# 0xmenna/spmv-scpa

Hardware: AMD Instinct MI355X
Metric: fp64 SpMV GFLOP/s + achieved HBM GB/s (% of roofline), 1/2/4/8 MI355X (higher is better)
Workload: dtype f64

## Files before the change

### include/spmv_engine.h

```cpp
#ifndef SPMV_ENGINE_H
#define SPMV_ENGINE_H

#include <stddef.h>
#include <stdint.h>

#include "csr.h"
#include "hll.h"

#ifdef __cplusplus
extern "C" {
#endif

typedef struct spmv_launch_opts {
    int waves_per_block;
    int group;
    int variant;
    int reserved[5];
} spmv_launch_opts;

int spmv_device_count(void);
int spmv_set_device(int device);
int spmv_get_device(void);
int spmv_device_info(int device, char *name, size_t len, int *compute_units,
                     size_t *hbm_bytes);
// ... 229 lines not shown
                      const spmv_trsv_plan *second, const double *d_scale,
                      double tol, int maxit, int check_every, void *d_work,
                      size_t work_bytes, spmv_cg_info *info, void *stream);

int64_t spmv_bicgstab_work_bytes(int M, int k);
int spmv_csr_bicgstab(const spmv_csr_dev *A, const spmv_launch_opts *opts,
                      int k, const double *d_B, int64_t ldb, double *d_X,
                      int64_t ldx, const double *d_minv,
                      double tol, int maxit, int check_every,
                      void *d_work, size_t work_bytes,
                      spmv_cg_info *info, void *stream);
int spmv_hll_bicgstab(const spmv_hll_dev *H, const spmv_launch_opts *opts,
                      int k, const double *d_B, int64_t ldb, double *d_X,
                      int64_t ldx, const double *d_minv,
                      double tol, int maxit, int check_every,
                      void *d_work, size_t work_bytes,
                      spmv_cg_info *info, void *stream);

typedef struct spmv_cgls_info {
    int status;
    int iterations;
    double ss;
    double atb;
    double rr;
} spmv_cgls_info;

int64_t spmv_cgls_work_bytes(int M, int N, int k);
int spmv_csr_cgls(const spmv_csr_dev *A, const spmv_csr_dev *AT,
                  const spmv_launch_opts *opts, int k,
                  const double *d_B, int64_t ldb, double *d_X, int64_t ldx,
                  double damp, double tol, int maxit, int check_every,
                  void *d_work, size_t work_bytes,
                  spmv_cgls_info *info, void *stream);
int spmv_hll_cgls(const spmv_hll_dev *H, const spmv_hll_dev *HT,
                  const spmv_launch_opts *opts, int k,
                  const double *d_B, int64_t ldb, double *d_X, int64_t ldx,
                  double damp, double tol, int maxit, int check_every,
                  void *d_work, size_t work_bytes,
                  spmv_cgls_info *info, void *stream);

typedef struct spmv_minres_info {
    int status;
    int iterations;
    double pp;
    double bn2;
    double rr;
    double bb;
} spmv_minres_info;

int64_t spmv_minres_work_bytes(int M, int k);
int spmv_csr_minres(const spmv_csr_dev *A, const spmv_launch_opts *opts, int k,
                    const double *d_B, int64_t ldb, double *d_X, int64_t ldx,
                    const double *d_minv, double tol, int maxit,
                    int check_every, void *d_work, size_t work_bytes,
                    spmv_minres_info *info, void *stream);
int spmv_hll_minres(const spmv_hll_dev *H, const spmv_launch_opts *opts, int k,
                    const double *d_B, int64_t ldb, double *d_X, int64_t ldx,
                    const double *d_minv, double tol, int maxit,
                    int check_every, void *d_work, size_t work_bytes,
                    spmv_minres_info *info, void *stream);
int spmv_debug_sqrt(const double *d_in, double *d_out, int64_t n, void *stream);

int spmv_csr_autotune(spmv_csr_dev *A, const double *d_x, double *d_y,
                      int allow_panels, int *best_kernel, double *best_ms);
int spmv_hll_autotune(spmv_hll_dev *H, const double *d_x, double *d_y,
                      int allow_panels, int *best_kernel, double *best_ms);

int spmv_csr_tune_times(const spmv_csr_dev *A, double *ms, int n);
int spmv_hll_tune_times(const spmv_hll_dev *H, double *ms, int n);
int spmv_csr_tune_log(const spmv_csr_dev *A, char *buf, size_t len);
int spmv_hll_tune_log(const spmv_hll_dev *H, char *buf, size_t len);

int spmv_live_handles(void);
long spmv_ignored_releases(void);
void spmv_set_debug(int on);
uint64_t spmv_handle_generation(const void *handle);
void spmv_csr_release_checked(spmv_csr_dev *A, uint64_t generation);
void spmv_hll_release_checked(spmv_hll_dev *H, uint64_t generation);

const char *spmv_version(void);
int spmv_csr_debug_stale_arrivals(spmv_csr_dev *A);
int spmv_hll_debug_stale_arrivals(spmv_hll_dev *H);

int spmv_hip_build_version(void);
int spmv_hip_runtime_version(void);
const char *spmv_build_flavour(void);

#ifdef __cplusplus
}
#endif
#endif
```

### spmv_scpa_amd/csrc/engine.hip

```cpp
#include <algorithm>
#include <cmath>
#include <functional>
#include <mutex>
#include <stdio.h>
#include <stdlib.h>
#include <string.h>
#include <string>
#include <thread>
#include <time.h>
#include <unordered_map>
#include <vector>

#include "err.h"
#include "hip_common.h"
#include "hip_csr.h"
#include "hip_hll.h"
#include "mat_ref.h"
#include "spmv_synth.h"
#include "stream_table.h"
#include "transpose_plan.h"
#include "trsv_plan.h"
#include "tune_blocked.h"
#include "utils.h"

// ... 51 lines not shown
    } while (0)

struct panels_ops {
    static void free(spmv_panels *p) { panels_free(p); }
    static void set_chain(spmv_panels *p, int v) { panels_set_chain(p, v); }
    static void set_waves(spmv_panels *p, int v) { panels_set_waves(p, v); }
    static void set_order(spmv_panels *p, int v) { panels_set_order(p, v); }
    static int balanced_tile_rows(int M, int max_rows) {
        return panels_balanced_tile_rows(M, max_rows);
    }
    static const char *build_phases(void) { return panels_last_build_phases(); }
    static double now_s(void) {
        struct timespec t;
        clock_gettime(CLOCK_MONOTONIC, &t);
        return (double)t.tv_sec + 1e-9 * (double)t.tv_nsec;
    }
};

struct tune_log {
    std::string text;
    void operator()(const char *line) {
        text += line;
        text += '\n';
    }
    char *release(void) const { return strdup(text.c_str()); }
};

extern "C" {

const char *spmv_version(void) { return "spmv_scpa_amd 0.7 gfx950"; }

int spmv_hip_build_version(void) { return HIP_VERSION; }
int spmv_hip_runtime_version(void) {
    int v = 0;
    return hipRuntimeGetVersion(&v) == hipSuccess ? v : -EIO;
}

const char *spmv_build_flavour(void) {
#ifdef SPMV_ABLATIONS
    return "ablations";
#else
    return "product";
#endif
}

int spmv_live_handles(void) {
    std::lock_guard<std::mutex> g(live().mu);
    return (int)live().handles.size();
}

long spmv_ignored_releases(void) {
    std::lock_guard<std::mutex> g(live().mu);
    return live().ignored;
}

void spmv_set_debug(int on) {
    std::lock_guard<std::mutex> g(live().mu);
    live().debug = on ? 1 : 0;
}

uint64_t spmv_handle_generation(const void *handle) {
    std::lock_guard<std::mutex> g(live().mu);
    auto it = live().handles.find(handle);
    return it == live().handles.end() ? 0 : it->second;
}

static int stale_arrivals(unsigned long long *cnt, int n, spmv_panels *P) {
    if (cnt && n > 0)
        HIP_RET(hipMemset(cnt, 0x01, (size_t)n * sizeof(unsigned long long)));
    else
        n = 0;
    const int p = panels_debug_stale_arrivals(P);
    return p < 0 ? p : n + p;
}

int spmv_csr_debug_stale_arrivals(spmv_csr_dev *A) {
    HANDLE_OK(A);
    return stale_arrivals(A->seg_count, A->n_rowblk, A->panels);
}

int spmv_hll_debug_stale_arrivals(spmv_hll_dev *H) {
    HANDLE_OK(H);
    return stale_arrivals(H->wide_cnt, H->n_wide_seg, H->panels);
}

void set_csr_waves_per_block(int waves) {
    g_csr_waves = waves < 1 ? 0 : (waves > 16 ? 16 : waves);
}

void set_hll_waves_per_block(int waves) {
    g_hll_waves = waves < 1 ? 0 : (waves > 16 ? 16 : waves);
}


int spmv_device_count(void) {
    int n = 0;
    if (hipGetDeviceCount(&n) != hipSuccess)
        return 0;
    return n;
}

int spmv_set_device(int device) {
    if (spmv_device_count() == 0)
        return -ENODEV;
    HIP_RET(hipSetDevice(device));
    return 0;
}

int spmv_get_device(void) {
    int d = 0;
    if (spmv_device_count() == 0)
        return -ENODEV;
    HIP_RET(hipGetDevice(&d));
    return d;
}

int spmv_device_info(int device, char *name, size_t len, int *compute_units,
                     size_t *hbm_bytes) {
    if (spmv_device_count() == 0)
        return -ENODEV;
    hipDeviceProp_t p;
    HIP_RET(hipGetDeviceProperties(&p, device));
    if (name && len)
        snprintf(name, len, "%s (%s)", p.name, p.gcnArchName);
    if (compute_units)
        *compute_units = p.multiProcessorCount;
    if (hbm_bytes)
        *hbm_bytes = p.totalGlobalMem;
    return 0;
}

int spmv_device_pci_bus_id(int device, char *buf, size_t len) {
    if (!buf || len < 16)
        return -EINVAL;
    if (spmv_device_count() == 0)
        return -ENODEV;
    HIP_RET(hipDeviceGetPCIBusId(buf, (int)len, device));
    return 0;
}

int spmv_dev_mem_info(size_t *free_bytes, size_t *total_bytes) {
    if (spmv_device_count() == 0)
        return -ENODEV;
    size_t f = 0, t = 0;
    HIP_RET(hipMemGetInfo(&f, &t));
    if (free_bytes)
        *free_bytes = f;
    if (total_bytes)
        *total_bytes = t;
    return 0;
}

int spmv_dev_malloc(void **dptr, size_t bytes) {
    if (!dptr)
        return -EINVAL;
    *dptr = NULL;
    if (spmv_device_count() == 0)
        return -ENODEV;
    HIP_RET(hipMalloc(dptr, bytes ? bytes : 16));
    return 0;
}

int spmv_dev_free(void *dptr) {
    if (!dptr)
        return 0;
    HIP_RET(hipFree(dptr));
// ... 2920 lines not shown
```

### spmv_scpa_amd/csrc/hip_common.h

```cpp
#ifndef SPMV_HIP_COMMON_H
#define SPMV_HIP_COMMON_H

#include <errno.h>
#include <hip/hip_runtime.h>
#include <stdint.h>
#include <type_traits>

#include "spmv_engine.h"

#define WAVE 64
#define NUM_XCD 8
#define XCD_GROUP 32
#define HACK HACK_SIZE

static inline unsigned grouped_grid(unsigned n) {
    return (n + NUM_XCD * XCD_GROUP - 1) / (NUM_XCD * XCD_GROUP) * NUM_XCD *
           XCD_GROUP;
}

static inline int hip_errno(hipError_t e) {
    switch (e) {
    case hipSuccess:
        return 0;
    case hipErrorNoDevice:
// ... 353 lines not shown
int bicgstab_solve(const cg_matrix *A, int k, const double *B, int64_t ldb,
                   double *X, int64_t ldx, const double *minv, double tol,
                   int maxit, int check_every, void *d_work, size_t work_bytes,
                   spmv_cg_info *info, hipStream_t s);

int64_t cgls_work_bytes(int M, int N, int k);
int cgls_solve(const cg_matrix *A, const cg_matrix *AT, int k, const double *B,
               int64_t ldb, double *X, int64_t ldx, double damp, double tol,
               int maxit, int check_every, void *d_work, size_t work_bytes,
               spmv_cgls_info *info, hipStream_t s);

int64_t minres_work_bytes(int M, int k);
int minres_solve(const cg_matrix *A, int k, const double *B, int64_t ldb,
                 double *X, int64_t ldx, const double *minv, double tol,
                 int maxit, int check_every, void *d_work, size_t work_bytes,
                 spmv_minres_info *info, hipStream_t s);
int minres_debug_sqrt(const double *d_in, double *d_out, int64_t n,
                      hipStream_t s);

int csr_diag(const spmv_csr_dev *A, double *out, int invert, hipStream_t s);
int hll_diag(const spmv_hll_dev *H, double *out, int invert, hipStream_t s);

int csr_transpose_dev(const spmv_csr_dev *A, spmv_csr_dev *T, hipStream_t s);
int csr_equal_dev(const spmv_csr_dev *X, const spmv_csr_dev *Y, int *pattern,
                  int *values, hipStream_t s);
void tr_scan(int *data, int64_t n, int *sums, hipStream_t s);

struct trsv_segment;
struct spmv_trsv_plan {
    int M, uplo, unit, levels, value_bytes, device;
    int widest_level;
    int64_t entries;
    int64_t zero_diag;
    int64_t bytes;
    int *level;
    int *order;
    int *level_ptr;
    int *rowptr;
    int *ja;
    void *as;
    double *diag;
    int *h_level_ptr;
    trsv_segment *segs;
    int n_segs;
};
int trsv_analyse_dev(const spmv_csr_dev *A, int uplo, int unit, int max_levels,
                     spmv_trsv_plan *P, hipStream_t s);
void trsv_free_dev(spmv_trsv_plan *P);
int trsv_solve_dev(const spmv_trsv_plan *P, int waves, int k, const double *B,
                   int64_t ldb, double *X, int64_t ldx, const double *scale,
                   hipStream_t s);

typedef int (*ic0_alloc_fn)(int M, int N, int64_t NZ, int value_bytes,
                            spmv_csr_dev **out);
int ic0_factor_dev(const spmv_csr_dev *A, double shift, int max_levels,
                   int waves, ic0_alloc_fn alloc, spmv_csr_dev **out,
                   spmv_ic0_info *info, hipStream_t s);

int csr_launch_kernel(const spmv_csr_dev *A, int kernel, int waves, int group,
                      int variant, const double *x, double *y, int r0, int r1,
                      hipStream_t s);
int hll_launch_kernel(const spmv_hll_dev *H, int kernel, int waves,
                      int variant, const double *x, double *y, int b0, int b1,
                      hipStream_t s);
int hll_fix_pads_dev(spmv_hll_dev *H, hipStream_t s);
int hll16_convert_dev(const spmv_hll_dev *src, spmv_hll_dev *dst,
                      unsigned *d_overflow, hipStream_t s);

int panels_from_csr(const spmv_csr_dev *A, int panel_cols, int sched,
                    int tile_rows, spmv_panels **out);
int panels_from_hll(const spmv_hll_dev *H, int panel_cols, int sched,
                    int tile_rows, spmv_panels **out);
int panels_from_csr_opts(const spmv_csr_dev *A, const spmv_panel_opts *o,
                         spmv_panels **out);
int panels_from_hll_opts(const spmv_hll_dev *H, const spmv_panel_opts *o,
                         spmv_panels **out);
void panels_get_opts(const spmv_panels *P, spmv_panel_opts *o);
int panels_is_sweep(const spmv_panels *P);
int panels_tile_rows(const spmv_panels *P);
int panels_is_chain(const spmv_panels *P);
void panels_set_chain(spmv_panels *P, int chain);
void panels_set_waves(spmv_panels *P, int waves);
int panels_debug_stale_arrivals(spmv_panels *P);
void panels_set_order(spmv_panels *P, int order);
int panels_waves(const spmv_panels *P);
void panels_fit_steps(const spmv_panels *P, int64_t *builtin, int64_t *fit);
void panels_set_fit_steps(spmv_panels *P, int64_t builtin, int64_t fit);
int panels_plan_kernel(const spmv_panels *P, int waves, int variant,
                       int *threads, int *groups, int *ordered);
int panels_launch(const spmv_panels *P, int M, int waves, int variant,
                  const double *x, double *y, hipStream_t s);
void panels_free(spmv_panels *p);
int64_t panels_nnz(const spmv_panels *P);
int panels_count(const spmv_panels *P);
int panels_steps(const spmv_panels *P);
int panels_tiles(const spmv_panels *P);
int panels_balanced_tile_rows(int M, int max_rows);
int panels_describe(const spmv_panels *P, char *buf, size_t len);
const char *panels_last_build_phases(void);
void panels_pool_begin(void);
void panels_pool_end(void);

extern int g_csr_waves;
extern int g_hll_waves;

#endif
```

### spmv_scpa_amd/csrc/panels.hip

```cpp
#include <algorithm>
#include <atomic>
#include <utility>
#include <hipcub/hipcub.hpp>
#include <stdio.h>
#include <string.h>
#include <vector>

#include <time.h>

#include "hip_common.h"
#include "panel_launch.h"
#include "panel_build.h"

#define SWEEP_SPIN_MAX 512
#define CNT_STRIDE 32
#define SWEEP_TAIL 16384

struct spmv_panels : panel_shape {
    int N;
    int shift;
    int reserve_cus;
    int pmajor;
    int64_t total;
    unsigned *ent;
    double *val;
    int64_t *bptr;
    int *blen;
    int64_t *cb;
    int *cpanel;
    int *nbk;
    int span;
    int residue;
    int bucket_order;
    int xcd_first[NUM_XCD + 1];
    int *phase_cnt;
    size_t phase_cnt_bytes;
    int nlong;
    int nlong_seg;
    int64_t long_nnz;
    int *long_row;
    int *long_ptr;
    int *long_ja;
    double *long_as;
    int2 *long_seg;
    int *long_seg0;
    double *long_part;
    unsigned long long *long_cnt;
    unsigned launch_epoch;
};

static hipError_t big_malloc(void **p, size_t bytes);
static void big_free(void *p);

template <bool POOLED> struct dev_block {
    void *p = NULL;
    dev_block() = default;
    dev_block(dev_block &&o) : p(o.p) { o.p = NULL; }
    dev_block &operator=(dev_block &&o) {
        std::swap(p, o.p);
        return *this;
    }
    ~dev_block() { reset(); }
    hipError_t alloc(size_t bytes) {
        return POOLED ? big_malloc(&p, bytes) : hipMalloc(&p, bytes);
    }
    void reset() {
        if (POOLED)
            big_free(p);
        else
            (void)hipFree(p);
        p = NULL;
    }
    template <typename T> T *as() const { return (T *)p; }
};
typedef dev_block<true> pooled_block;
typedef dev_block<false> plain_block;

void panels_free(spmv_panels *p) {
    if (!p)
        return;
    big_free(p->ent);
    big_free(p->val);
    (void)hipFree(p->cpanel);
    (void)hipFree(p->phase_cnt);
    (void)hipFree(p->bptr);
    (void)hipFree(p->blen);
    (void)hipFree(p->cb);
    (void)hipFree(p->nbk);
    (void)hipFree(p->long_row);
    (void)hipFree(p->long_ptr);
    (void)hipFree(p->long_ja);
    (void)hipFree(p->long_as);
    (void)hipFree(p->long_seg);
    (void)hipFree(p->long_seg0);
    (void)hipFree(p->long_part);
    (void)hipFree(p->long_cnt);
    free(p);
}

__host__ __device__ __forceinline__ uint64_t bucket_id(uint64_t tile,
                                                       uint64_t panel,
                                                       uint64_t panels,
                                                       uint64_t pm_grid) {
    return pm_grid ? ((tile / pm_grid) * panels + panel) * pm_grid + tile % pm_grid
                   : tile * panels + panel;
}

__device__ __forceinline__ bool in_sorted(const int *__restrict__ rows, int n,
                                          int row) {
    int lo = 0, hi = n;
    while (lo < hi) {
        const int mid = (lo + hi) >> 1;
        if (rows[mid] < row)
            lo = mid + 1;
        else
            hi = mid;
    }
    return lo < n && rows[lo] == row;
}
// ... 675 lines not shown

static int compact_lists(const panel_geometry &g, spmv_panels *P,
                         plain_block &span_block) {
    const int tiles = g.tiles, panels = g.panels;
    HIP_RET(hipMalloc((void **)&P->cb,
                      ((size_t)g.nbuckets + 1) * 2 * sizeof(int64_t)));
    HIP_RET(hipMalloc((void **)&P->cpanel,
                      ((size_t)g.nbuckets + 1) * sizeof(int)));
    HIP_RET(hipMalloc((void **)&P->nbk, ((size_t)tiles + 1) * sizeof(int)));
    HIP_RET(hipMemset(P->nbk, 0, ((size_t)tiles + 1) * sizeof(int)));
    if (tiles > 0) {
        HIP_RET(span_block.alloc((2 * (size_t)tiles + 1) * sizeof(int)));
        int *span = span_block.as<int>();
        HIP_RET(hipMemset(span + 2 * (size_t)tiles, 0, sizeof(int)));
        hipLaunchKernelGGL(k_tile_span, dim3((tiles + 255) / 256), dim3(256), 0,
                           0, tiles, panels, P->blen, span, span + tiles,
                           span + 2 * (size_t)tiles);
        HIP_RET(hipGetLastError());
        HIP_RET(hipMemcpy(&P->span, span + 2 * (size_t)tiles, sizeof(int),
                          hipMemcpyDeviceToHost));
        P->residue = P->bucket_order != 1 && P->span > 1 && P->span < panels;
        hipLaunchKernelGGL(k_compact_buckets, dim3((tiles + 255) / 256),
                           dim3(256), 0, 0, tiles, panels,
                           P->residue ? P->span : panels, P->bptr, P->blen, span,
                           span + tiles, P->cb, P->cpanel, P->nbk);
        hipLaunchKernelGGL(k_max_int, dim3(64), dim3(256), 0, 0, tiles, P->nbk,
                           P->nbk + tiles);
        HIP_RET(hipGetLastError());
    }
    HIP_RET(hipMemcpy(&P->max_nbk, P->nbk + tiles, sizeof(int),
                      hipMemcpyDeviceToHost));
    return 0;
}

static int bucket_totals(const panel_geometry &g, const int64_t *raw,
                         spmv_panels *P) {
    HIP_RET(hipMemcpy(&P->nnz, raw + g.nbuckets, sizeof(int64_t),
                      hipMemcpyDeviceToHost));
    HIP_RET(hipMemcpy(&P->total, P->bptr + g.nbuckets, sizeof(int64_t),
                      hipMemcpyDeviceToHost));
    return P->total + SWEEP_TAIL > (int64_t)3000000000LL ? -EOVERFLOW : 0;
}

static int place_entries(const panel_geometry &g, const uint64_t *skey,
                         const double *sval, const int64_t *raw,
                         spmv_panels *P) {
    const size_t m = (size_t)P->total + SWEEP_TAIL;
    HIP_RET(big_malloc((void **)&P->ent, m * sizeof(unsigned)));
    HIP_RET(big_malloc((void **)&P->val, m * sizeof(double)));
    HIP_RET(hipMemset(P->ent, 0, m * sizeof(unsigned)));
    HIP_RET(hipMemset(P->val, 0, m * sizeof(double)));
    if (P->nnz > 0) {
        const unsigned grid = (unsigned)((P->nnz + 255) / 256);
        hipLaunchKernelGGL(k_place, dim3(grid), dim3(256), 0, 0, P->nnz, g.shift,
                           g.rbits, skey, sval, raw, P->bptr, P->ent, P->val);
        HIP_RET(hipGetLastError());
        HIP_RET(hipDeviceSynchronize());
    }
    return 0;
}

static int count_chunk_steps(const panel_geometry &g, spmv_panels *P) {
    P->fit_steps[0] = P->fit_steps[1] = 0;
    panel_plan pl;
    if (g.nbuckets <= 0 || P->nnz <= 0 ||
        panel_launch_plan(*P, 0, 0, false, &pl) || pl.family != PANEL_SWEEP)
        return 0;
    plain_block sums;
    HIP_RET(sums.alloc(2 * sizeof(unsigned long long)));
    HIP_RET(hipMemset(sums.p, 0, 2 * sizeof(unsigned long long)));
    hipLaunchKernelGGL(k_chunk_steps, dim3(64), dim3(256), 0, 0,
                       (int64_t)g.nbuckets, P->blen, pl.k.threads * pl.k.q * 4,
                       PANEL_FIT_CHUNK, sums.as<unsigned long long>());
    HIP_RET(hipGetLastError());
    unsigned long long h[2] = {0, 0};
    HIP_RET(hipMemcpy(h, sums.p, sizeof h, hipMemcpyDeviceToHost));
    P->fit_steps[0] = (int64_t)h[0];
    P->fit_steps[1] = (int64_t)h[1];
    return 0;
}

static int alloc_phase_counters(const panel_geometry &g, spmv_panels *P) {
    const size_t rounds = ((size_t)g.tiles + g.grid - 1) / g.grid;
    P->phase_cnt_bytes = NUM_XCD * (rounds ? rounds : 1) * (size_t)g.panels *
                         CNT_STRIDE * sizeof(int);
    HIP_RET(hipMalloc((void **)&P->phase_cnt, P->phase_cnt_bytes));
    return 0;
}

struct build_scratch {
    pooled_block key[2], sv[2];
    pooled_block idx;
    pooled_block tmp;
    pooled_block flag;
    plain_block count;
    plain_block raw, padded;
    plain_block span;
    ~build_scratch() {
        for (int k = 0; k < 2; ++k) {
            key[k].reset();
            sv[k].reset();
        }
        idx.reset();
        tmp.reset();
        flag.reset();
        count.reset();
        raw.reset();
        padded.reset();
        span.reset();
    }
};

static int build_stages(const panel_geometry &g, const build_src &s,
                        spmv_panels *P) {
    int rc;
    build_scratch b;
    const bool hll = !s.irp;
    int64_t n_sort = s.slots;
    uint64_t *skey;
    double *sval;
    double tp[5] = {build_now_s(), 0, 0, 0, 0};

    if ((rc = long_rows_extract(P, s)))
        return rc;
    if (hll && s.slots > 0 &&
        (rc = hll_flag_kept(s, P, b.flag, b.count, &n_sort)))
        return rc;
    if ((rc = alloc_sort_buffers(n_sort, hll && n_sort != s.slots, b.key, b.sv,
                                 b.idx)))
        return rc;
    skey = b.key[0].as<uint64_t>();
    sval = b.sv[0].as<double>();
    if (s.slots > 0) {
        rc = hll ? keys_from_hll(g, s, n_sort, b.flag, b.count, b.idx, skey, sval)
                 : keys_from_csr(g, s, P, skey, sval);
        if (rc)
            return rc;
        tp[1] = build_now_s();
        b.idx.reset();
        if ((rc = sort_keys(g, n_sort, b.key, b.sv, b.tmp, &skey, &sval)))
            return rc;
    }
    tp[2] = build_now_s();
    if ((rc = bucket_tables(g, n_sort, skey, P, b.raw, b.padded)))
        return rc;
    if (!g.sweep && (rc = compact_lists(g, P, b.span)))
        return rc;
    if ((rc = bucket_totals(g, b.raw.as<int64_t>(), P)))
        return rc;
    tp[3] = build_now_s();
    if ((rc = place_entries(g, skey, sval, b.raw.as<int64_t>(), P)))
        return rc;
    if ((rc = g.sweep ? alloc_phase_counters(g, P) : balance_xcd_ranges(P)))
        return rc;
    if (g.sweep && (rc = count_chunk_steps(g, P)))
        return rc;
    tp[4] = build_now_s();
    snprintf(g_build_phases, sizeof g_build_phases,
             "%lld of %lld slots sorted: alloc+keys %.3f s, sort %.3f, bucket "
             "tables %.3f, place %.3f",
             (long long)n_sort, (long long)s.slots,
             tp[1] > 0 ? tp[1] - tp[0] : 0.0, tp[1] > 0 ? tp[2] - tp[1] : 0.0,
             tp[3] - tp[2], tp[4] - tp[3]);
    return 0;
}

static int panels_build(int N, const build_src &s, const spmv_panel_opts *o,
                        spmv_panels **out) {
    *out = NULL;
    spmv_panel_opts dflt;
    spmv_panel_opts_default(&dflt);
    if (!o)
        o = &dflt;
    long long tall_rows = 0;
#ifdef SPMV_ABLATIONS
    if (const char *e = getenv("SPMV_ABL_SWEEP_TILE_ROWS")) {
        const long long v = atoll(e) / 32 * 32;
        if (v >= 32 && v < (1 << 20))
            tall_rows = v;
    }
#endif
    panel_geometry g;
    int rc = panel_build_plan(s.M, N, s.slots, *o,
                              g_panel_sched.load(std::memory_order_relaxed),
                              device_cus, tall_rows, &g);
    if (rc)
        return rc;
    spmv_panels *P = (spmv_panels *)calloc(1, sizeof *P);
    if (!P)
        return -ENOMEM;
    P->N = N;
    P->shift = g.shift;
    P->panels = g.panels;
    P->tile_rows = g.tile_rows;
    P->tiles = g.tiles;
    P->sweep = g.sweep;
    P->chain = g.chain;
    P->grid = g.grid;
    P->wgs_per_cu = g.wgs_per_cu;
    P->reserve_cus = g.reserve_cus;
    P->pmajor = g.pmajor;
    P->lds_min = o->lds_min;
    P->bucket_order = o->bucket_order;
    P->det = g.det;
    P->order = g.order;
    g_build_phases[0] = 0;
    rc = build_stages(g, s, P);
    if (rc) {
        panels_free(P);
        return rc;
    }
    *out = P;
    return 0;
}

__device__ __forceinline__ void phase_arrive(int *cnt, int n = 1) {
    __hip_atomic_fetch_add(cnt, n, __ATOMIC_RELAXED, __HIP_MEMORY_SCOPE_AGENT);
}

__device__ __forceinline__ bool phase_wait(const int *cnt, int want, int spin) {
    for (int i = 0; i < spin; ++i) {
        if (__hip_atomic_load(cnt, __ATOMIC_RELAXED, __HIP_MEMORY_SCOPE_AGENT) >=
            want)
            return true;
        __builtin_amdgcn_s_sleep(8);
    }
    return false;
}

#define WAVE_RING 32
__device__ __forceinline__ void wg_arrive(int *ring, int q, int waves,
                                          int *cnt_q) {
    const int old = atomicAdd(&ring[q & (WAVE_RING - 1)], 1);
    if (old == waves - 1) {
        atomicExch(&ring[q & (WAVE_RING - 1)], 0);
        phase_arrive(cnt_q);
    }
}

typedef unsigned u32x4 __attribute__((ext_vector_type(4)));
typedef double f64x2 __attribute__((ext_vector_type(2)));


#ifndef SPMV_DET_SLEEP
#define SPMV_DET_SLEEP 1
#endif
__device__ __forceinline__ void det_wait(int *turn, int want) {
    while (__hip_atomic_load(turn, __ATOMIC_ACQUIRE,
                             __HIP_MEMORY_SCOPE_WORKGROUP) != want) {
#if SPMV_DET_SLEEP > 0
        __builtin_amdgcn_s_sleep(SPMV_DET_SLEEP);
#endif
    }
}

__device__ __forceinline__ void det_have(double v) {
    asm volatile("" ::"v"(v));
}

__device__ __forceinline__ void det_pass(int *turn, int next) {
    __hip_atomic_store(turn, next, __ATOMIC_RELEASE,
                       __HIP_MEMORY_SCOPE_WORKGROUP);
}

template <int Q> struct sweep_chunk {
    u32x4 en[Q];
    f64x2 va[Q], vb[Q];
    int live[Q];
    int p;
    int pa;
    bool first, last;
};

template <int NT, int Q, int ABL = 0, bool DET = false>
__global__ void __launch_bounds__(NT)
    k_tiles_sweep(int M, int tile_rows, int tiles, int panels, int shift,
                  int lag, int spin, int stagger, int pmajor, unsigned total,
                  const int64_t *__restrict__ bptr,
                  const int *__restrict__ blen,
                  const unsigned *__restrict__ tent,
                  const double *__restrict__ tval,
                  const double *__restrict__ x, double *__restrict__ y,
                  int *phase_cnt) {
    extern __shared__ double ytile[];
    __shared__ int wave_done[WAVE_RING];
    constexpr int WAVES = NT / WAVE;
    constexpr unsigned CH = NT * Q * 4;
    const int tid = threadIdx.x;
    const int grid = gridDim.x;
    const int xcd = blockIdx.x % NUM_XCD;
    const int n_x = grid / NUM_XCD + (xcd < (grid % NUM_XCD) ? 1 : 0);
    const int rounds = (tiles + grid - 1) / grid;
    int *cnt = phase_cnt + (size_t)xcd * rounds * panels * CNT_STRIDE;
    const unsigned lowmask = (ABL & 2) ? 1023u : (1u << shift) - 1u;
    __shared__ int det_turn;
    int det_seq = tid / WAVE;
    if (tid < WAVE_RING)
        wave_done[tid] = 0;
    if (tid == 0)
        det_turn = 0;
    bool synced = true;

    for (int r = 0; r < rounds; ++r) {
        const int t = r * grid + blockIdx.x;
        const int q0 = r * panels;
        if (t >= tiles) {
            if (tid == 0)
                for (int p = 0; p < panels; ++p)
                    phase_arrive(cnt + (size_t)(q0 + p) * CNT_STRIDE);
            continue;
        }
        for (int i = tid; i < ((ABL & 8) && tile_rows > 16384 ? 16384 : tile_rows);
             i += NT)
            ytile[i] = 0.0;
        __syncthreads();

        const int64_t bbase = pmajor ? (int64_t)q0 * grid + blockIdx.x
                                     : (int64_t)t * panels;
        const int64_t bstep = pmajor ? grid : 1;
        auto bp = [&](int p) { return bptr[bbase + (int64_t)p * bstep]; };
        auto bl = [&](int p) { return blen[bbase + (int64_t)p * bstep]; };
        bool ready = !(lag > 0 && q0 >= lag);

        const int poff = stagger ? (int)((long long)xcd * panels / NUM_XCD) : 0;
        int fp = 0, fpa = poff % panels;
        unsigned fk = (unsigned)bp(fpa), fe = fk + (unsigned)bl(fpa);
        unsigned fb = fk;
        bool ffirst = true;

        auto fill = [&](sweep_chunk<Q> &c) {
            c.p = fp;
            c.pa = fpa;
            c.first = ffirst;
            c.last = fk + CH >= fe;
#pragma unroll
            for (int g = 0; g < Q; ++g) {
                unsigned blk = fk + ((unsigned)g * NT + (tid & ~(WAVE - 1))) * 4u;
                const unsigned lane = tid & (WAVE - 1);
                c.live[g] = (int)(fe - blk) - (int)lane;
                if (pmajor && blk >= fe && fe > fb)
                    blk = fb;
                if (ABL & 4)
                    blk &= 0x3FFFu;
                c.en[g] = __builtin_nontemporal_load(
                    (const u32x4 *)(tent + blk + lane * 4u));
                c.va[g] = __builtin_nontemporal_load(
                    (const f64x2 *)(tval + blk + lane * 2u));
                c.vb[g] = __builtin_nontemporal_load(
                    (const f64x2 *)(tval + blk + 128u + lane * 2u));
            }
            if (fp < panels) {
                if (!c.last) {
                    fk += CH;
                    ffirst = false;
                } else {
                    fp += 1;
                    fpa = fpa + 1 < panels ? fpa + 1 : 0;
                    ffirst = true;
                    if (fp < panels) {
                        fk = (unsigned)bp(fpa);
                        fe = fk + (unsigned)bl(fpa);
                    } else {
                        fk = total;
                        fe = total;
                    }
                    fb = fk;
                }
            }
        };

        auto step = [&](sweep_chunk<Q> &c, sweep_chunk<Q> &f) {
            const int q = q0 + c.p;
            if (c.first && !ready && synced)
                synced = phase_wait(cnt + (size_t)(q - lag) * CNT_STRIDE, n_x,
                                    spin);
            const double *xp = x + ((int64_t)c.pa << shift);
            double pr[Q][4], w[Q][4];
            unsigned rr[Q][4];
            int on[Q];
#pragma unroll
            for (int g = 0; g < Q; ++g) {
                on[g] = c.live[g];
#pragma unroll
                for (int u = 0; u < 4; ++u) {
                    const unsigned col = 64 * u < on[g] ? (c.en[g][u] & lowmask) : 0u;
                    pr[g][u] = xp[col];
                    rr[g][u] = c.en[g][u] >> shift;
                    if (ABL & 8)
                        rr[g][u] &= 16383u;
                }
                w[g][0] = c.va[g][0];
                w[g][1] = c.va[g][1];
                w[g][2] = c.vb[g][0];
                w[g][3] = c.vb[g][1];
            }
            const bool last = c.last;
            const int qn = (last && lag > 0 && q + 1 >= lag) ? q + 1 - lag : 0;
            const int polled = __hip_atomic_load(cnt + (size_t)qn * CNT_STRIDE,
                                                 __ATOMIC_RELAXED,
                                                 __HIP_MEMORY_SCOPE_AGENT);
            fill(f);
            if (DET)
                det_wait(&det_turn, det_seq);
#pragma unroll
            for (int g = 0; g < Q; ++g)
#pragma unroll
                for (int u = 0; u < 4; ++u) {
                    const double prod = pr[g][u] * w[g][u];
                    if (ABL & 1) {
                        if (64 * u < on[g] && prod == 1.2345e300)
                            ytile[rr[g][u]] = 1.0;
                    } else if (64 * u < on[g]) {
                        unsafeAtomicAdd(&ytile[rr[g][u]], prod);
                    }
                }
            if (DET) {
                det_pass(&det_turn, det_seq + 1);
                det_seq += WAVES;
            }
            if (last) {
                ready = lag <= 0 || q + 1 < lag || polled >= n_x;
                if ((tid & (WAVE - 1)) == 0)
                    wg_arrive(wave_done, q, WAVES, cnt + (size_t)q * CNT_STRIDE);
            }
        };

        sweep_chunk<Q> A, B, C;
        fill(A);
        fill(B);
        for (;;) {
            step(A, C);
            if (B.p >= panels)
                break;
            step(B, A);
            if (C.p >= panels)
                break;
            step(C, B);
            if (A.p >= panels)
                break;
        }
        __syncthreads();
        const int64_t row0 = (int64_t)t * tile_rows;
        for (int i = tid; i < tile_rows && row0 + i < M; i += NT)
            __builtin_nontemporal_store(ytile[(ABL & 8) ? (i & 16383) : i],
                                        y + row0 + i);
        __syncthreads();
    }
}


__device__ __forceinline__ bool tile_of_workgroup(int tiles_hw,
                                                  const xcd_ranges &xr, int &t) {
    int t_end;
    if (tiles_hw > 0) {
        t = (int)blockIdx.x;
        t_end = tiles_hw;
    } else if (tiles_hw < 0) {
        const int G = (-tiles_hw) >> 24, k = blockIdx.x / NUM_XCD;
        t = ((k / G) * NUM_XCD + (int)(blockIdx.x % NUM_XCD)) * G + k % G;
        t_end = (-tiles_hw) & 0xffffff;
    } else {
        t = xr.first[blockIdx.x % NUM_XCD] + (int)(blockIdx.x / NUM_XCD);
        t_end = xr.first[blockIdx.x % NUM_XCD + 1];
    }
    return t < t_end;
}

template <int NT, int Q>
__device__ __forceinline__ void load_chunk(sweep_chunk<Q> &c, unsigned k0,
                                           unsigned e, const unsigned *tent,
                                           const double *tval, int tid) {
    const unsigned lane = tid & (WAVE - 1);
    const unsigned wbase = (tid & ~(WAVE - 1)) * 4u;
#pragma unroll
    for (int g = 0; g < Q; ++g) {
        const unsigned blk = k0 + (unsigned)g * NT * 4u + wbase;
        c.live[g] = (int)(e - blk) - (int)lane;
        c.en[g] = __builtin_nontemporal_load(
            (const u32x4 *)(tent + blk + lane * 4u));
        c.va[g] = __builtin_nontemporal_load(
            (const f64x2 *)(tval + blk + lane * 2u));
        c.vb[g] = __builtin_nontemporal_load(
            (const f64x2 *)(tval + blk + 128u + lane * 2u));
    }
}

template <int NT, int Q, bool DET, typename Next>
__device__ __forceinline__ void add_chunk(const sweep_chunk<Q> &c,
                                          const double *xp, unsigned lowmask,
                                          int shift, double *ytile,
                                          int *det_turn, int &det_seq,
                                          Next next) {
    double pr[Q][4], w[Q][4];
    unsigned rr[Q][4];
    int on[Q];
#pragma unroll
    for (int g = 0; g < Q; ++g) {
        on[g] = c.live[g];
#pragma unroll
        for (int u = 0; u < 4; ++u) {
            const unsigned col = 64 * u < on[g] ? (c.en[g][u] & lowmask) : 0u;
            pr[g][u] = xp[col];
            rr[g][u] = c.en[g][u] >> shift;
        }
        w[g][0] = c.va[g][0];
        w[g][1] = c.va[g][1];
        w[g][2] = c.vb[g][0];
        w[g][3] = c.vb[g][1];
    }
    next();
    if (DET) {
#pragma unroll
        for (int g = 0; g < Q; ++g)
#pragma unroll
            for (int u = 0; u < 4; ++u) {
                pr[g][u] *= w[g][u];
                w[g][u] = 1.0;
                det_have(pr[g][u]);
            }
        det_wait(det_turn, det_seq);
    }
#pragma unroll
    for (int g = 0; g < Q; ++g)
#pragma unroll
        for (int u = 0; u < 4; ++u)
            if (64 * u < on[g])
                unsafeAtomicAdd(&ytile[rr[g][u]],
                                DET ? pr[g][u] : pr[g][u] * w[g][u]);
    if (DET) {
        det_pass(det_turn, det_seq + 1);
// ... 130 lines not shown

template <auto Kernel> static int allow_big_lds(void) {
    static std::atomic<unsigned long long> done{0};
    int dev = 0;
    HIP_RET(hipGetDevice(&dev));
    const unsigned long long bit = 1ull << (dev & 63);
    if (!(done.load(std::memory_order_acquire) & bit)) {
        HIP_RET(hipFuncSetAttribute(reinterpret_cast<const void *>(Kernel),
                                    hipFuncAttributeMaxDynamicSharedMemorySize,
                                    BIG_LDS_BYTES));
        done.fetch_or(bit, std::memory_order_release);
    }
    return 0;
}

#ifdef SPMV_ABLATIONS
constexpr bool ABLATIONS = true;
#else
constexpr bool ABLATIONS = false;
#endif

template <typename K> struct tile_kernel {
    K launch;
    int (*allow)(void);
};
template <auto Kernel>
constexpr tile_kernel<decltype(Kernel)> tile_kernel_of = {
    Kernel, &allow_big_lds<Kernel>};
using sweep_fn = decltype(&k_tiles_sweep<256, 1>);
using chain_fn = decltype(&k_tiles_chain<256, 1>);
using step_fn = decltype(&k_tiles_step<256, 1>);

template <int... I>
static const tile_kernel<sweep_fn> &sweep_kernel(int row,
                                                 std::integer_sequence<int, I...>) {
    static const tile_kernel<sweep_fn> rows[] = {tile_kernel_of<&k_tiles_sweep<
        PANEL_SWEEP_KERNELS[I].threads, PANEL_SWEEP_KERNELS[I].q,
        PANEL_SWEEP_KERNELS[I].abl, PANEL_SWEEP_KERNELS[I].det != 0>>...};
    return rows[row];
}
template <int... I>
static const tile_kernel<chain_fn> &chain_kernel(int row,
                                                 std::integer_sequence<int, I...>) {
    static const tile_kernel<chain_fn> rows[] = {tile_kernel_of<&k_tiles_chain<
        PANEL_CHAIN_KERNELS[I].threads, PANEL_CHAIN_KERNELS[I].q,
        PANEL_CHAIN_KERNELS[I].det != 0>>...};
    return rows[row];
}
template <int... I>
static const tile_kernel<step_fn> &step_kernel(int row,
                                               std::integer_sequence<int, I...>) {
    static const tile_kernel<step_fn> rows[] = {tile_kernel_of<&k_tiles_step<
        PANEL_STEP_KERNELS[I].threads, PANEL_STEP_KERNELS[I].q,
        PANEL_STEP_KERNELS[I].det != 0>>...};
    return rows[row];
}

static int panels_launch_tiles(const spmv_panels *P, int M, int waves,
                               int variant, const double *x, double *y,
                               hipStream_t s);

int panels_launch(const spmv_panels *P, int M, int waves, int variant,
                  const double *x, double *y, hipStream_t s) {
    const int rc = panels_launch_tiles(P, M, waves, variant, x, y, s);
    if (rc || !P->nlong)
        return rc;
    hipLaunchKernelGGL(k_long_rows, dim3(P->nlong_seg), dim3(256), 0, s,
                       P->long_seg, P->nlong_seg, P->long_row, P->long_ptr,
                       P->long_seg0, P->long_ja, P->long_as, x, y, P->long_part,
                       P->long_cnt, next_launch_epoch(&P->launch_epoch));
    return hip_errno(hipGetLastError());
}

static int panels_launch_tiles(const spmv_panels *P, int M, int waves,
                               int variant, const double *x, double *y,
                               hipStream_t s) {
    if (!P)
        return -EINVAL;
    if (M == 0)
        return 0;
    panel_plan pl;
    if (int rc = panel_launch_plan(*P, waves, variant, ABLATIONS, &pl))
        return rc;
    (void)hipGetLastError();
    if (pl.launches == 0)
        return 0;
    const int row = panel_plan_row(pl, ABLATIONS);
    const dim3 grid(pl.grid), block(pl.k.threads);
    if (pl.family == PANEL_SWEEP) {
        HIP_RET(hipMemsetAsync(P->phase_cnt, 0, P->phase_cnt_bytes, s));
        const auto &k = sweep_kernel(
            row, std::make_integer_sequence<int, panel_sweep_kernels(ABLATIONS)>{});
        if (int rc = k.allow())
            return rc;
        hipLaunchKernelGGL(k.launch, grid, block, pl.lds, s, M, P->tile_rows,
                           P->tiles, P->panels, P->shift, pl.lag,
                           SWEEP_SPIN_MAX, pl.stagger, P->pmajor,
                           (unsigned)P->total, P->bptr, P->blen, P->ent, P->val,
                           x, y, P->phase_cnt);
        return hip_errno(hipGetLastError());
    }
    if (!P->cb || !P->cpanel || !P->nbk)
        return -EINVAL;
    xcd_ranges xr;
    memcpy(xr.first, P->xcd_first, sizeof xr.first);
    if (pl.family == PANEL_CHAIN) {
        const auto &k = chain_kernel(
            row, std::make_integer_sequence<int, PANEL_CHAIN_PRODUCT>{});
        if (int rc = k.allow())
            return rc;
        hipLaunchKernelGGL(k.launch, grid, block, pl.lds, s, M, P->tile_rows,
                           P->panels, P->shift, (unsigned)P->total,
                           pl.order_arg, xr, P->cb, P->cpanel, P->nbk, P->ent,
                           P->val, x, y);
        return hip_errno(hipGetLastError());
    }
    const auto &k =
        step_kernel(row, std::make_integer_sequence<int, PANEL_STEP_PRODUCT>{});
    if (int rc = k.allow())
        return rc;
    for (int p = 0; p < pl.launches; ++p)
        hipLaunchKernelGGL(k.launch, grid, block, pl.lds, s, M, P->tile_rows,
                           P->panels, P->shift, p, pl.order_arg, xr, P->cb,
                           P->cpanel, P->nbk, P->ent, P->val, x, y);
    return hip_errno(hipGetLastError());
}

int panels_from_csr_opts(const spmv_csr_dev *A, const spmv_panel_opts *o,
                         spmv_panels **out) {
    const build_src s = {A->M, 0, A->NZ, A->irp, NULL, 0, A->ja, A->as, NULL};
    return panels_build(A->N, s, o, out);
}

int panels_from_hll_opts(const spmv_hll_dev *H, const spmv_panel_opts *o,
                         spmv_panels **out) {
    if (H->index_bytes == 2)
        return -ENOTSUP;
    if (H->slots > 0 && !H->padmask)
        return -ENODATA;
    const build_src s = {H->M,  H->nb, H->slots, NULL,      H->off,
                         H->col_major, H->ja, H->as, H->padmask};
    return panels_build(H->N, s, o, out);
}

extern "C" void spmv_panel_opts_default(spmv_panel_opts *o) {
    if (!o)
        return;
    memset(o, 0, sizeof *o);
    o->struct_size = (int)sizeof *o;
    o->sched = -1;
    o->sweep_layout = -1;
}

int panels_from_csr(const spmv_csr_dev *A, int panel_cols, int sched,
                    int tile_rows, spmv_panels **out) {
    spmv_panel_opts o;
    spmv_panel_opts_default(&o);
    o.sched = sched;
    o.panel_cols = panel_cols;
    o.tile_rows = tile_rows;
    return panels_from_csr_opts(A, &o, out);
}

int panels_from_hll(const spmv_hll_dev *H, int panel_cols, int sched,
                    int tile_rows, spmv_panels **out) {
    spmv_panel_opts o;
    spmv_panel_opts_default(&o);
    o.sched = sched;
    o.panel_cols = panel_cols;
    o.tile_rows = tile_rows;
    return panels_from_hll_opts(H, &o, out);
}

void panels_get_opts(const spmv_panels *P, spmv_panel_opts *o) {
    spmv_panel_opts_default(o);
    o->sched = P->sweep ? 1 : P->chain ? 2 : 0;
    o->panel_cols = 1 << P->shift;
    o->tile_rows = P->sweep ? 0 : P->tile_rows;
    o->sweep_wgs_per_cu = P->sweep ? P->wgs_per_cu : 0;
    o->reserve_cus = P->reserve_cus;
    o->lds_min = P->lds_min;
    o->tile_order = P->order;
    o->sweep_layout = P->pmajor;
    o->bucket_order = P->bucket_order;
    o->deterministic = P->det ? 1 : 2;
}

int panels_describe(const spmv_panels *P, char *buf, size_t len) {
    if (!P || !buf || !len)
        return -EINVAL;
    if (P->sweep)
        snprintf(buf, len,
                 "sweep tiles=%d x %d rows, panels=%d x 2^%d cols, grid=%d "
                 "(%d wg/cu, reserve %d), buckets %s-major, waves=%d",
                 P->tiles, P->tile_rows, P->panels, P->shift, P->grid,
                 P->wgs_per_cu, P->reserve_cus, P->pmajor ? "panel" : "tile",
                 P->waves_hint);
    else
        snprintf(buf, len,
                 "%s tiles=%d x %d rows, panels=%d x 2^%d cols, <=%d buckets "
                 "per tile (span %d, %s order), tile order %d, waves=%d",
                 P->chain ? "chain" : "steps", P->tiles, P->tile_rows,
                 P->panels, P->shift, P->max_nbk, P->span,
                 P->residue ? "residue" : "ascending", P->order,
                 P->waves_hint);
    if (P->det) {
        const size_t at = strlen(buf);
        snprintf(buf + at, len - at, ", deterministic");
    }
    if (P->nlong) {
        const size_t at = strlen(buf);
        snprintf(buf + at, len - at,
                 "; %d long row(s) beside the copy (%lld entries, %d segments)",
                 P->nlong, (long long)P->long_nnz, P->nlong_seg);
    }
    return 0;
}

int panels_is_sweep(const spmv_panels *P) { return P ? P->sweep : 0; }
int panels_is_chain(const spmv_panels *P) { return P ? P->chain : 0; }
void panels_set_chain(spmv_panels *P, int chain) {
    if (P && !P->sweep)
        P->chain = chain != 0;
}
int panels_waves(const spmv_panels *P) { return P ? P->waves_hint : 0; }
void panels_set_order(spmv_panels *P, int order) {
    if (P && !P->sweep && order >= 0 && order <= 2)
        P->order = order;
}
void panels_set_waves(spmv_panels *P, int waves) {
    if (P)
        P->waves_hint = waves > 0 ? waves : 0;
}
int panels_tile_rows(const spmv_panels *P) { return P ? P->tile_rows : 0; }
void panels_fit_steps(const spmv_panels *P, int64_t *builtin, int64_t *fit) {
    *builtin = P ? P->fit_steps[0] : 0;
    *fit = P ? P->fit_steps[1] : 0;
}
void panels_set_fit_steps(spmv_panels *P, int64_t builtin, int64_t fit) {
    if (P) {
        P->fit_steps[0] = builtin > 0 ? builtin : 0;
        P->fit_steps[1] = fit > 0 ? fit : 0;
    }
}
int panels_plan_kernel(const spmv_panels *P, int waves, int variant,
                       int *threads, int *groups, int *ordered) {
    panel_plan pl;
    if (!P)
        return -EINVAL;
    if (int rc = panel_launch_plan(*P, waves, variant, ABLATIONS, &pl))
        return rc;
    *threads = pl.k.threads;
    *groups = pl.k.q;
    *ordered = pl.k.det;
    return 0;
}

int panels_debug_stale_arrivals(spmv_panels *P) {
    if (!P || !P->nlong)
        return 0;
    HIP_RET(hipMemset(P->long_cnt, 0x01,
                      (size_t)P->nlong * sizeof(unsigned long long)));
    return P->nlong;
}

int64_t panels_nnz(const spmv_panels *P) {
    return P ? P->nnz + P->long_nnz : 0;
}
int panels_count(const spmv_panels *P) { return P ? P->panels : 0; }
int panels_steps(const spmv_panels *P) {
    return P ? (P->sweep || P->chain ? 1 : P->max_nbk) : 0;
}
int panels_tiles(const spmv_panels *P) { return P ? P->tiles : 0; }
```

Baseline: 454.2.

## Self-reset sweep phase counters in-kernel to drop per-launch memset

The sweep kernel now resets its phase counters itself. The last wave on each XCD to leave, detected through an extra per-XCD done counter, zeroes the counters, so the host no longer issues a hipMemsetAsync before every launch; a host flag forces a memset only after a launch error. The ytile zeroing is folded into the y store loop so it is done once per round rather than at the start of each round. The masked-lane loads are also made branchless. This adds an atomic exit protocol and carries a risk of stale counters if a launch aborts partway through.

```diff
diff --git a/include/spmv_engine.h b/include/spmv_engine.h
--- a/include/spmv_engine.h
+++ b/include/spmv_engine.h
@@ -335,6 +335,11 @@
 int spmv_csr_debug_stale_arrivals(spmv_csr_dev *A);
 int spmv_hll_debug_stale_arrivals(spmv_hll_dev *H);
 
+int spmv_csr_debug_stale_phases(spmv_csr_dev *A, int mark);
+int spmv_hll_debug_stale_phases(spmv_hll_dev *H, int mark);
+int spmv_csr_debug_phase_words(spmv_csr_dev *A);
+int spmv_hll_debug_phase_words(spmv_hll_dev *H);
+
 int spmv_hip_build_version(void);
 int spmv_hip_runtime_version(void);
 const char *spmv_build_flavour(void);
diff --git a/spmv_scpa_amd/csrc/engine.hip b/spmv_scpa_amd/csrc/engine.hip
--- a/spmv_scpa_amd/csrc/engine.hip
+++ b/spmv_scpa_amd/csrc/engine.hip
@@ -157,6 +157,26 @@
 int spmv_hll_debug_stale_arrivals(spmv_hll_dev *H) {
     HANDLE_OK(H);
     return stale_arrivals(H->wide_cnt, H->n_wide_seg, H->panels);
+}
+
+int spmv_csr_debug_stale_phases(spmv_csr_dev *A, int mark) {
+    HANDLE_OK(A);
+    return panels_debug_stale_phases(A->panels, mark);
+}
+
+int spmv_hll_debug_stale_phases(spmv_hll_dev *H, int mark) {
+    HANDLE_OK(H);
+    return panels_debug_stale_phases(H->panels, mark);
+}
+
+int spmv_csr_debug_phase_words(spmv_csr_dev *A) {
+    HANDLE_OK(A);
+    return panels_debug_phase_words(A->panels);
+}
+
+int spmv_hll_debug_phase_words(spmv_hll_dev *H) {
+    HANDLE_OK(H);
+    return panels_debug_phase_words(H->panels);
 }
 
 void set_csr_waves_per_block(int waves) {
diff --git a/spmv_scpa_amd/csrc/hip_common.h b/spmv_scpa_amd/csrc/hip_common.h
--- a/spmv_scpa_amd/csrc/hip_common.h
+++ b/spmv_scpa_amd/csrc/hip_common.h
@@ -459,6 +459,8 @@
 void panels_set_chain(spmv_panels *P, int chain);
 void panels_set_waves(spmv_panels *P, int waves);
 int panels_debug_stale_arrivals(spmv_panels *P);
+int panels_debug_stale_phases(spmv_panels *P, int mark);
+int panels_debug_phase_words(const spmv_panels *P);
 void panels_set_order(spmv_panels *P, int order);
 int panels_waves(const spmv_panels *P);
 void panels_fit_steps(const spmv_panels *P, int64_t *builtin, int64_t *fit);
diff --git a/spmv_scpa_amd/csrc/panels.hip b/spmv_scpa_amd/csrc/panels.hip
--- a/spmv_scpa_amd/csrc/panels.hip
+++ b/spmv_scpa_amd/csrc/panels.hip
@@ -35,6 +35,7 @@
     int xcd_first[NUM_XCD + 1];
     int *phase_cnt;
     size_t phase_cnt_bytes;
+    int needs_reset;
     int nlong;
     int nlong_seg;
     int64_t long_nnz;
@@ -876,9 +877,11 @@
 
 static int alloc_phase_counters(const panel_geometry &g, spmv_panels *P) {
     const size_t rounds = ((size_t)g.tiles + g.grid - 1) / g.grid;
-    P->phase_cnt_bytes = NUM_XCD * (rounds ? rounds : 1) * (size_t)g.panels *
+    P->phase_cnt_bytes = NUM_XCD * ((rounds ? rounds : 1) * (size_t)g.panels + 1) *
                          CNT_STRIDE * sizeof(int);
     HIP_RET(hipMalloc((void **)&P->phase_cnt, P->phase_cnt_bytes));
+    HIP_RET(hipMemset(P->phase_cnt, 0, P->phase_cnt_bytes));
+    P->needs_reset = 0;
     return 0;
 }
 
@@ -1032,6 +1035,39 @@
     }
 }
 
+__device__ __forceinline__ void sweep_leave(int *cnt, int words, int *done,
+                                            int n_x, int lane) {
+    int mine = 0;
+    if (lane == 0) {
+        int old = __hip_atomic_fetch_add(done, 1, __ATOMIC_RELAXED,
+                                         __HIP_MEMORY_SCOPE_AGENT);
+        if ((unsigned)old >= (unsigned)n_x) {
+            old = __hip_atomic_load(done, __ATOMIC_RELAXED,
+                                    __HIP_MEMORY_SCOPE_AGENT);
+            for (;;) {
+                if ((unsigned)old < (unsigned)n_x) {
+                    old = __hip_atomic_fetch_add(done, 1, __ATOMIC_RELAXED,
+                                                 __HIP_MEMORY_SCOPE_AGENT);
+                    break;
+                }
+                if (__hip_atomic_compare_exchange_strong(
+                        done, &old, 1, __ATOMIC_RELAXED, __ATOMIC_RELAXED,
+                        __HIP_MEMORY_SCOPE_AGENT)) {
+                    old = 0;
+                    break;
+                }
+            }
+        }
+        mine = old + 1;
+    }
+    if (__builtin_amdgcn_readfirstlane(mine) != n_x)
+        return;
+    for (int i = lane; i < words; i += WAVE)
+        cnt[(size_t)i * CNT_STRIDE] = 0;
+    if (lane == 0)
+        *done = 0;
+}
+
 typedef unsigned u32x4 __attribute__((ext_vector_type(4)));
 typedef double f64x2 __attribute__((ext_vector_type(2)));
 
@@ -1095,6 +1131,9 @@
         det_turn = 0;
     bool synced = true;
 
+    constexpr bool ALIASED = (ABL & 8) != 0;
+    const int acc_rows = ALIASED && tile_rows > 16384 ? 16384 : tile_rows;
+
     for (int r = 0; r < rounds; ++r) {
         const int t = r * grid + blockIdx.x;
         const int q0 = r * panels;
@@ -1104,10 +1143,11 @@
                     phase_arrive(cnt + (size_t)(q0 + p) * CNT_STRIDE);
             continue;
         }
-        for (int i = tid; i < ((ABL & 8) && tile_rows > 16384 ? 16384 : tile_rows);
-             i += NT)
-            ytile[i] = 0.0;
-        __syncthreads();
+        if (r == 0) {
+            for (int i = tid; i < acc_rows; i += NT)
+                ytile[i] = 0.0;
+            __syncthreads();
+        }
 
         const int64_t bbase = pmajor ? (int64_t)q0 * grid + blockIdx.x
                                      : (int64_t)t * panels;
@@ -1132,16 +1172,17 @@
                 unsigned blk = fk + ((unsigned)g * NT + (tid & ~(WAVE - 1))) * 4u;
                 const unsigned lane = tid & (WAVE - 1);
                 c.live[g] = (int)(fe - blk) - (int)lane;
-                if (pmajor && blk >= fe && fe > fb)
-                    blk = fb;
+                const bool masked = (pmajor != 0) & (blk >= fe);
+                blk = (masked & (fe > fb)) ? fb : blk;
+                const unsigned at = masked ? 0u : lane;
                 if (ABL & 4)
                     blk &= 0x3FFFu;
                 c.en[g] = __builtin_nontemporal_load(
-                    (const u32x4 *)(tent + blk + lane * 4u));
+                    (const u32x4 *)(tent + blk + at * 4u));
                 c.va[g] = __builtin_nontemporal_load(
-                    (const f64x2 *)(tval + blk + lane * 2u));
+                    (const f64x2 *)(tval + blk + at * 2u));
                 c.vb[g] = __builtin_nontemporal_load(
-                    (const f64x2 *)(tval + blk + 128u + lane * 2u));
+                    (const f64x2 *)(tval + blk + 128u + at * 2u));
             }
             if (fp < panels) {
                 if (!c.last) {
@@ -1235,11 +1276,28 @@
         }
         __syncthreads();
         const int64_t row0 = (int64_t)t * tile_rows;
-        for (int i = tid; i < tile_rows && row0 + i < M; i += NT)
-            __builtin_nontemporal_store(ytile[(ABL & 8) ? (i & 16383) : i],
-                                        y + row0 + i);
+        if (ALIASED) {
+            for (int i = tid; i < tile_rows && row0 + i < M; i += NT)
+                __builtin_nontemporal_store(ytile[i & 16383], y + row0 + i);
+            __syncthreads();
+            for (int i = tid; i < acc_rows; i += NT)
+                ytile[i] = 0.0;
+        } else {
+            for (int i = tid; i < tile_rows; i += NT) {
+                if (row0 + i < M)
+                    __builtin_nontemporal_store(ytile[i], y + row0 + i);
+                ytile[i] = 0.0;
+            }
+        }
         __syncthreads();
     }
+    __builtin_amdgcn_s_waitcnt(0);
+    __syncthreads();
+    if (tid < WAVE)
+        sweep_leave(cnt, rounds * panels,
+                    phase_cnt + ((size_t)NUM_XCD * rounds * panels + xcd) *
+                                    CNT_STRIDE,
+                    n_x, tid);
 }
 
 
@@ -1536,23 +1594,31 @@
     panel_plan pl;
     if (int rc = panel_launch_plan(*P, waves, variant, ABLATIONS, &pl))
         return rc;
-    (void)hipGetLastError();
+    int *needs_reset = const_cast<int *>(&P->needs_reset);
+    if (hipGetLastError() != hipSuccess && P->sweep)
+        __atomic_store_n(needs_reset, 1, __ATOMIC_RELAXED);
     if (pl.launches == 0)
         return 0;
     const int row = panel_plan_row(pl, ABLATIONS);
     const dim3 grid(pl.grid), block(pl.k.threads);
     if (pl.family == PANEL_SWEEP) {
-        HIP_RET(hipMemsetAsync(P->phase_cnt, 0, P->phase_cnt_bytes, s));
         const auto &k = sweep_kernel(
             row, std::make_integer_sequence<int, panel_sweep_kernels(ABLATIONS)>{});
         if (int rc = k.allow())
             return rc;
+        if (__atomic_load_n(needs_reset, __ATOMIC_RELAXED)) {
+            HIP_RET(hipMemsetAsync(P->phase_cnt, 0, P->phase_cnt_bytes, s));
+            __atomic_store_n(needs_reset, 0, __ATOMIC_RELAXED);
+        }
         hipLaunchKernelGGL(k.launch, grid, block, pl.lds, s, M, P->tile_rows,
                            P->tiles, P->panels, P->shift, pl.lag,
                            SWEEP_SPIN_MAX, pl.stagger, P->pmajor,
                            (unsigned)P->total, P->bptr, P->blen, P->ent, P->val,
                            x, y, P->phase_cnt);
-        return hip_errno(hipGetLastError());
+        const int rc = hip_errno(hipGetLastError());
+        if (rc)
+            __atomic_store_n(needs_reset, 1, __ATOMIC_RELAXED);
+        return rc;
     }
     if (!P->cb || !P->cpanel || !P->nbk)
         return -EINVAL;
@@ -1718,6 +1784,37 @@
     return P->nlong;
 }
 
+static size_t phase_words(const spmv_panels *P) {
+    return P && P->sweep && P->phase_cnt
+               ? P->phase_cnt_bytes / (CNT_STRIDE * sizeof(int))
+               : 0;
+}
+
+int panels_debug_stale_phases(spmv_panels *P, int mark) {
+    const size_t n = phase_words(P);
+    if (!n)
+        return 0;
+    HIP_RET(hipDeviceSynchronize());
+    HIP_RET(hipMemset(P->phase_cnt, 0x01, P->phase_cnt_bytes));
+    if (mark)
+        __atomic_store_n(&P->needs_reset, 1, __ATOMIC_RELAXED);
+    return (int)n;
+}
+
+int panels_debug_phase_words(const spmv_panels *P) {
+    const size_t n = phase_words(P);
+    if (!n)
+        return 0;
+    HIP_RET(hipDeviceSynchronize());
+    std::vector<int> h(n * CNT_STRIDE);
+    HIP_RET(hipMemcpy(h.data(), P->phase_cnt, P->phase_cnt_bytes,
+                      hipMemcpyDeviceToHost));
+    int left = 0;
+    for (size_t i = 0; i < n; ++i)
+        left += h[i * CNT_STRIDE] != 0;
+    return left;
+}
+
 int64_t panels_nnz(const spmv_panels *P) {
     return P ? P->nnz + P->long_nnz : 0;
 }
```

New measurement: 448.9. -1.2%, worse.
